# HybridRobotics/ilqr-iterative-tasks

Measured on AMD Instinct MI355X. Metric: batched iLQR iterations/s (n=6,m=2,N=20), higher is better.
Workload: dtype f64

## Files before the change

ilqr_iterative_tasks_amd/csrc/i2lqr_abi.hip:

```cpp
#include <hip/hip_runtime.h>
#include <dlfcn.h>
#include <rccl/rccl.h>

#include <atomic>
#include <cmath>
#include <cstdarg>
#include <cstdio>
#include <cstdlib>
#include <cstring>
#include <mutex>
#include <new>
#include <unordered_set>

#include "../../include/i2lqr.h"
#include "i2lqr_devcfg.hpp"
#include "i2lqr_geometry.hpp"
#include "i2lqr_group.h"
#include "i2lqr_lane.hpp"
#include "i2lqr_select.hpp"
#include "i2lqr_wave.hpp"

#include "i2lqr_lane12.h"

#define I2LQR_DRY_RUN_LANE 1
// ... 354 lines not shown
      return;
    }
  }
  f(std::false_type());
}

template <class T>
IterArgs<T> iter_args(int64_t B, int n_iters, int early_exit, void* X, void* U, const void* x_term,
                      void* lamb, const void* obs, void* cost, void* K, void* k, int32_t* iters,
                      int32_t* status) {
  IterArgs<T> a;
  a.B = B; a.n_iters = n_iters; a.early_exit = early_exit;
  a.X = (T*)X; a.U = (T*)U; a.x_term = (const T*)x_term; a.lamb = (T*)lamb; a.obs = (const T*)obs;
  a.cost = (T*)cost; a.K = (T*)K; a.k = (T*)k; a.iters = iters; a.status = status;
  a.dbg = nullptr;
  a.count = nullptr; a.count_max = 0; a.max_total = 0; a.set_stride = 0;
  return a;
}

template <class T, class Sys> struct Launch {
  static constexpr int n = Sys::n, m = Sys::m, LANES = 64;
  using Cfg = DevCfg<T, n, m>;

  static size_t lds_bytes(int N) { return (size_t)Layout<Sys>(N).total * sizeof(T) * (64 / LANES); }
  static size_t fstep_lds_bytes(int N) {
    return (size_t)Layout<Sys>(N, true).total * sizeof(T) * (64 / LANES);
  }
  static constexpr bool kHasFstep = Sys::n <= 6;
  static unsigned grid(int64_t B) { return (unsigned)((B + (64 / LANES) - 1) / (64 / LANES)); }

  static int prepare(i2lqr_handle* h) {
    h->lanes = LANES;
    h->lds_bytes = lds_bytes(h->cfg.N);
    if (h->lds_bytes > h->geo.max_dyn_lds)
      return fail(I2LQR_ERR_UNSUPPORTED, "horizon %d needs %zu B of LDS per wavefront (> %zu KiB)",
                  h->cfg.N, h->lds_bytes, h->geo.max_dyn_lds / 1024);
    if (h->lds_bytes > h->geo.default_dyn_lds)
      for (const void* kernel :
           {(const void*)k_iterate<T, Sys, LANES, false>, (const void*)k_iterate<T, Sys, LANES, true>,
            (const void*)k_backward<T, Sys, LANES, false>, (const void*)k_backward<T, Sys, LANES, true>,
            (const void*)k_forward<T, Sys, LANES, false>, (const void*)k_forward<T, Sys, LANES, true>,
            (const void*)k_rollout<T, Sys, LANES, false>, (const void*)k_rollout<T, Sys, LANES, true>})
        HIP_TRY(hipFuncSetAttribute(kernel, hipFuncAttributeMaxDynamicSharedMemorySize,
                                    (int)h->lds_bytes));
    return I2LQR_OK;
  }

  static int iterate(i2lqr_handle* h, int64_t B, int n_iters, int early_exit, void* X, void* U,
                     const void* x_term, void* lamb, const void* obs, void* cost, void* K, void* k,
                     int32_t* iters, int32_t* status, hipStream_t s) {
    const Cfg c = make_dev_cfg<T, n, m>(h->cfg);
    IterArgs<T> a = iter_args<T>(B, n_iters, early_exit, X, U, x_term, lamb, obs, cost, K, k, iters,
                                 status);
#ifdef I2LQR_STAMPS
    a.dbg = (unsigned long long*)h->ws;
#endif
    const char* why = "";
    const FusedKernel fk = select_fused(h, B, early_exit != 0, &why);
    if (t_epi && (fk == K_GROUP || fk == K_GROUP16 || fk == K_GROUP_WS)) {
      a.qfun = t_epi->qfun;
      a.outer_iter = t_epi->outer_iter;
      a.max_relax_iter = t_epi->max_relax_iter;
      a.cost_it = (T*)t_epi->cost_it;
      if (t_epi->best_idx) {
        a.pick_part = (MinPair<T>*)t_epi->part;
        a.pick_ticket = h->ticket + h->ticket_next.fetch_add(1, std::memory_order_relaxed) %
                                        i2lqr_handle::kTickets;
        a.best_idx = t_epi->best_idx;
        a.best_cost = (T*)t_epi->best_cost;
      }
      t_epi->fused = true;
    }
    switch (fk) {
      case K_INVALID:
        return fail(I2LQR_ERR_UNSUPPORTED, "%s", why);
      case K_SPEC:
      case K_SPEC16:
        if constexpr (m == 2 && n + m <= 8) {
          HIP_TRY(group_spec_iterate<T>(h->cfg, a, s, fk == K_SPEC16 ? 16 : 8));
          return I2LQR_OK;
        }
        break;
      case K_GROUP:
        if constexpr (m == 2 && n + m <= 8) {
          HIP_TRY(group_iterate<T>(h->cfg, a, s));
          return I2LQR_OK;
        }
        break;
      case K_GROUP16:
        if constexpr (m == 2 && n + m <= 8) {
          HIP_TRY(group16_iterate<T>(h->cfg, a, s, h->opt_group_overlap != 0));
          return I2LQR_OK;
        }
        break;
      case K_GROUP_WS:
        if constexpr (m == 2 && n + m <= 8) {
          HIP_TRY(group_iterate_ws<T>(h->cfg, a, h->ws, s));
          return I2LQR_OK;
        }
        break;
      case K_QUAD:
        if constexpr (n + m == 16) {
          HIP_TRY(quad_iterate<T>(h->cfg, a, h->ws, s));
          return I2LQR_OK;
        }
        break;
      case K_WAVE:
        break;
    }
    const size_t lds_f = fstep_lds_bytes(h->cfg.N);
    const int64_t waves_per_cu = (grid(B) + h->geo.cus - 1) / h->geo.cus;
    const bool fstep = kHasFstep && lds_f <= h->geo.default_dyn_lds &&
                       (h->opt_fstep >= 0 ? h->opt_fstep != 0
                                          : waves_per_cu * lds_f <= h->geo.lds_per_cu - 10 * 1024);
    if constexpr (kHasFstep) {
      if (fstep) {
        with_weights(c.flags, [&](auto W) {
          hipLaunchKernelGGL((k_iterate<T, Sys, LANES, W, true>), dim3(grid(B)), dim3(64), lds_f, s, c, a);
        });
        HIP_TRY(hipGetLastError());
        return I2LQR_OK;
      }
    }
    with_weights(c.flags, [&](auto W) {
      hipLaunchKernelGGL((k_iterate<T, Sys, LANES, W>), dim3(grid(B)), dim3(64), h->lds_bytes, s, c, a);
    });
    HIP_TRY(hipGetLastError());
    return I2LQR_OK;
  }
  static int names_pair(i2lqr_handle*, int64_t, int) { return 0; }
  static int solve_chained(i2lqr_handle* h, int64_t L, int k, void* X, void* U, const void* x_term,
                           void* lamb, const void* obs, void* cost, void* K, void* kk, int32_t* iters,
                           int32_t* status, hipStream_t s) {
    if constexpr (m == 2 && n + m <= 8) {
      if (h->opt_spec == 0 || h->opt_group == 8 || h->opt_group == 64 ||
          !group_spec_chain_supported(h->cfg, L))
        return fail(I2LQR_ERR_UNSUPPORTED, "chains run on the sixteen-lane speculative kernel: a "
                    "bicycle plant with Q = R = 0, at most %lld chains, a horizon whose three-wavefront "
                    "buffers fit a CU's LDS (solve the chain steps one after the other instead)",
                    (long long)h->geo.scaled(512));
      IterArgs<T> a = iter_args<T>(L, h->cfg.max_iter, 1, X, U, x_term, lamb, obs, cost, K, kk, iters,
                                   status);
      a.chain_len = k;
      HIP_TRY(group_spec_chain<T>(h->cfg, a, s));
// ... 949 lines not shown
      if (cfg->Q[i * I2LQR_MAX_N + j] != cfg->Q[j * I2LQR_MAX_N + i] ||
          cfg->Qt[i * I2LQR_MAX_N + j] != cfg->Qt[j * I2LQR_MAX_N + i]) lane_ok = false;
  for (int a = 0; a < cfg->m; a++)
    for (int b = 0; b < cfg->m; b++)
      if (cfg->R[a * I2LQR_MAX_M + b] != cfg->R[b * I2LQR_MAX_M + a]) lane_ok = false;
  int64_t from;
  switch (cfg->system_id) {
    case I2LQR_SYS_BICYCLE4:
    case I2LQR_SYS_BICYCLE6:
      from = weights ? kLaneFromWeights
                     : (early_exit ? lane_from(*cfg).solve : lane_from(*cfg).iterate);
      break;
    case I2LQR_SYS_QUAD12: {
      const LaneFrom q = kLaneFromQuad[cfg->N <= 31 ? 0 : 1][cfg->dtype == I2LQR_F64 ? 0 : 1];
      from = weights ? kLaneFromWeights : (early_exit ? q.solve : q.iterate);
      if (cfg->dtype != I2LQR_F64 && weights) lane_ok = false;
      break;
    }
    default: return fail(I2LQR_ERR_INVALID, "unknown system_id %d", cfg->system_id);
  }
  from = device_geometry().scaled_from(from);
  if (!lane_ok || B < from) return I2LQR_LAYOUT_PROBLEM_MAJOR;
  return B % 64 == 0 ? I2LQR_LAYOUT_BATCH_TILED : I2LQR_LAYOUT_BATCH_MINOR;
}

int i2lqr_set_compaction(i2lqr_handle* h, int64_t min_batch) {
  if (!h) return fail(I2LQR_ERR_INVALID, "null handle");
  if (h->cfg.layout == I2LQR_LAYOUT_PROBLEM_MAJOR && min_batch > 0)
    return fail(I2LQR_ERR_UNSUPPORTED, "compaction applies to the batch-minor / batch-tiled layouts");
  h->compact_min_batch = min_batch < 0 ? -1 : min_batch;
  return I2LQR_OK;
}

int i2lqr_set_option(i2lqr_handle* h, const char* name, int64_t value) {
  if (!h || !name) return fail(I2LQR_ERR_INVALID, "null handle or option name");
  if (value < -1 || value > 0x7fffffff) return fail(I2LQR_ERR_INVALID, "option value out of range");
  const int v = (int)value;
  if (!strcmp(name, "defer_states")) h->opt_defer = v < 0 ? -1 : (v != 0);
  else if (!strcmp(name, "reroll_nominal")) h->opt_reroll = v < 0 ? -1 : (v != 0);
  else if (!strcmp(name, "lds_gain_steps")) h->opt_lds_steps = v;
  else if (!strcmp(name, "merge_inputs")) h->opt_merge = v < 0 ? -1 : (v != 0);
  else if (!strcmp(name, "checkpoint_states")) h->opt_ckpt = v < 0 ? -1 : (v != 0);
  else if (!strcmp(name, "stagger")) h->opt_stagger = v;
  else if (!strcmp(name, "per_step_jacobians")) h->opt_fstep = v < 0 ? -1 : (v != 0);
  else if (!strcmp(name, "wave_tail")) h->wave_tail = v < 0 ? -1 : (v > 65536 ? 65536 : v);
  else if (!strcmp(name, "first_chunk")) h->opt_first_chunk = v < 1 ? -1 : (v > 1024 ? 1024 : v);
  else if (!strcmp(name, "helper_wavefront")) h->opt_pair = v < 0 ? -1 : (v != 0);
  else if (!strcmp(name, "state_buffers")) h->opt_two_x = v < 0 ? -1 : (v != 0);
  else if (!strcmp(name, "chunk_step")) h->opt_chunk_step = v < 1 ? -1 : (v > 1024 ? 1024 : v);
  else if (!strcmp(name, "fused_compaction")) h->opt_fuse = v < 0 ? -1 : (v != 0);
  else if (!strcmp(name, "final_round")) h->opt_final_round = v < 0 ? -1 : (v > 20 ? 20 : v);
  else if (!strcmp(name, "speculate")) h->opt_spec = v < 0 ? -1 : (v != 0);
  else if (!strcmp(name, "group_workspace")) h->opt_group_ws = v < 0 ? -1 : (v != 0);
  else if (!strcmp(name, "group_overlap")) h->opt_group_overlap = v < 0 ? -1 : (v != 0);
  else if (!strcmp(name, "debug_self_test")) {
#ifdef I2LQR_DEBUG
    unsigned long long* w = i2lqr::debug_trap_word();
    double* buf = nullptr;
    HIP_TRY(hipMalloc((void**)&buf, 8 * sizeof(double)));
    hipLaunchKernelGGL(k_debug_self_test, dim3(1), dim3(64), 0, (hipStream_t)0, buf, w);
    const int rc = debug_check(I2LQR_OK, nullptr);
    (void)hipFree(buf);
    return rc;
#else
    return fail(I2LQR_ERR_UNSUPPORTED, "\"debug_self_test\" exists in the index-checked debug build "
                "only (make -C ilqr_iterative_tasks_amd/csrc debug)");
#endif
  }
  else if (!strcmp(name, "group_lanes")) {
    if (v != -1 && v != 8 && v != 16 && v != 64)
      return fail(I2LQR_ERR_INVALID, "\"group_lanes\" is 8, 16, 64 or -1");
    h->opt_group = v;
  }
  else return fail(I2LQR_ERR_INVALID, "unknown option '%s'", name);
  return I2LQR_OK;
}

static const char* kernel_name(const i2lqr_handle* h, int64_t B, bool early_exit) {
  if (!h) return "";
  if (h->cfg.layout != I2LQR_LAYOUT_PROBLEM_MAJOR) {
    if (h->cfg.system_id == I2LQR_SYS_QUAD12) return "k_lane_iterate_rows";
    const auto pair = [&](auto L) {
      return L.names_pair(const_cast<i2lqr_handle*>(h), B, early_exit ? 1 : 0);
    };
    return dispatch(h, pair) == 1 ? "k_lane_iterate_pair" : "k_lane_iterate";
  }
  switch (select_fused(h, B, early_exit, nullptr)) {
    case K_SPEC: return "k_group_spec";
    case K_SPEC16: return "k_group_spec (sixteen lanes)";
    case K_GROUP: return "k_group_iterate";
    case K_GROUP16: return "k_group_iterate (sixteen lanes)";
    case K_GROUP_WS: return "k_group_iterate (workspace form)";
    case K_QUAD: return "k_quad_iterate";
    case K_WAVE: return "k_iterate";
    default: return "unsupported";
  }
}

const char* i2lqr_iterate_kernel(const i2lqr_handle* h, int64_t B) { return kernel_name(h, B, false); }
const char* i2lqr_solve_kernel(const i2lqr_handle* h, int64_t B) { return kernel_name(h, B, true); }

int i2lqr_set_workspace(i2lqr_handle* h, void* workspace, int64_t bytes) {
  if (!h) return fail(I2LQR_ERR_INVALID, "null handle");
  if (bytes < 0 || (bytes > 0 && !workspace) || ((uintptr_t)workspace & 15))
    return fail(I2LQR_ERR_INVALID, "workspace must be a 16-byte aligned device pointer");
  h->ws = workspace;
  h->ws_bytes = bytes;
// ... 558 lines not shown
```

ilqr_iterative_tasks_amd/csrc/i2lqr_group.h:

```cpp
#pragma once
#include <hip/hip_runtime.h>

#include "../../include/i2lqr.h"
#include "i2lqr_wave.hpp"

namespace i2lqr {

bool group_supported(const i2lqr_config& cfg);
template <class T> hipError_t group_iterate(const i2lqr_config& cfg, const IterArgs<T>& a,
                                            hipStream_t stream);

constexpr int64_t kGroup16Batch = 4096;
bool group16_supported(const i2lqr_config& cfg);
template <class T> hipError_t group16_iterate(const i2lqr_config& cfg, const IterArgs<T>& a,
                                              hipStream_t stream, bool overlap = true);

constexpr int64_t kGroupWsBatch = 4096;
constexpr int64_t kGroupWsTop = 8192;
constexpr int64_t kGroupWsTopF32 = 7168;
inline int64_t group_ws_top(const i2lqr_config& cfg) {
  return cfg.dtype == I2LQR_F64 ? kGroupWsTop : kGroupWsTopF32;
}
int64_t group_workspace_bytes(const i2lqr_config& cfg, int64_t B);
template <class T> hipError_t group_iterate_ws(const i2lqr_config& cfg, const IterArgs<T>& a,
                                               void* ws, hipStream_t stream);

bool group_spec_supported(const i2lqr_config& cfg, int lanes);
template <class T> hipError_t group_spec_iterate(const i2lqr_config& cfg, const IterArgs<T>& a,
                                                 hipStream_t stream, int lanes);
bool group_spec_chain_supported(const i2lqr_config& cfg, int64_t chains);
template <class T> hipError_t group_spec_chain(const i2lqr_config& cfg, const IterArgs<T>& a,
                                               hipStream_t stream);
bool group_spec_tail_supported(const i2lqr_config& cfg);
template <class T> hipError_t group_spec_tail(const i2lqr_config& cfg, const IterArgs<T>& a,
                                              hipStream_t stream);

bool quad_supported(const i2lqr_config& cfg);
int64_t quad_workspace_bytes(const i2lqr_config& cfg, int64_t B);
template <class T> hipError_t quad_iterate(const i2lqr_config& cfg, const IterArgs<T>& a, void* ws,
                                           hipStream_t stream);

}
```

ilqr_iterative_tasks_amd/csrc/i2lqr_group.hip:

```cpp
#include "i2lqr_group.h"

#include "i2lqr_devcfg.hpp"
#include "i2lqr_geometry.hpp"
#include "i2lqr_group.hpp"
#include "i2lqr_dryrun.hpp"

namespace i2lqr {

namespace {

template <class T, class Sys, int G = kGroup> size_t group_lds_bytes(int N) {
  return (size_t)GLayout<Sys, G>(N).wave_words() * sizeof(T);
}

template <auto Kernel> hipError_t raise_lds_limit(size_t lds) {
  if (lds <= device_geometry().default_dyn_lds) return hipSuccess;
  constexpr int kMaxDev = 64;
  static thread_local int raised_for[kMaxDev] = {};
  int dev = 0;
  hipError_t e = hipGetDevice(&dev);
  if (e != hipSuccess) return e;
  if (dev < 0 || dev >= kMaxDev || raised_for[dev] < (int)lds) {
    e = hipFuncSetAttribute((const void*)Kernel, hipFuncAttributeMaxDynamicSharedMemorySize,
                            (int)lds);
    if (e != hipSuccess) return e;
    if (dev >= 0 && dev < kMaxDev) raised_for[dev] = (int)lds;
  }
  return hipSuccess;
}

template <class T, class Sys, int H, int G = kGroup>
hipError_t launch_h(const i2lqr_config& cfg, const IterArgs<T>& a, hipStream_t s) {
  const auto c = make_dev_cfg<T, Sys::n, Sys::m>(cfg);
  const size_t lds = group_lds_bytes<T, Sys, G>(cfg.N);
  if (hipError_t e = raise_lds_limit<k_group_iterate<T, Sys, H, false, G>>(lds); e != hipSuccess)
    return e;
  constexpr int PW = 64 / G;
  const unsigned grid = (unsigned)((a.B + PW - 1) / PW);
  hipLaunchKernelGGL((k_group_iterate<T, Sys, H, false, G>), dim3(grid), dim3(64 * H), lds, s, c, a,
                     (T*)nullptr);
  return hipGetLastError();
}
template <class T, class Sys>
hipError_t launch16(const i2lqr_config& cfg, const IterArgs<T>& a, hipStream_t s, bool overlap) {
  const int64_t cus = device_geometry().cus;
#ifndef I2LQR_STAMPS
  if (overlap && (a.B + 3) / 4 <= cus) return launch_h<T, Sys, 3, 16>(cfg, a, s);
  if ((a.B + 3) / 4 <= 2 * cus) return launch_h<T, Sys, 2, 16>(cfg, a, s);
#endif
  return launch_h<T, Sys, 1, 16>(cfg, a, s);
}
template <class T, class Sys>
hipError_t launch_ws(const i2lqr_config& cfg, const IterArgs<T>& a, void* ws, hipStream_t s) {
  const auto c = make_dev_cfg<T, Sys::n, Sys::m>(cfg);
  const size_t lds = (size_t)GLayout<Sys>(cfg.N, true).wave_words() * sizeof(T);
  if (hipError_t e = raise_lds_limit<k_group_iterate<T, Sys, 1, true>>(lds); e != hipSuccess) return e;
  const unsigned grid = (unsigned)((a.B + kGroupsPerWave - 1) / kGroupsPerWave);
  hipLaunchKernelGGL((k_group_iterate<T, Sys, 1, true>), dim3(grid), dim3(64), lds, s, c, a, (T*)ws);
  return hipGetLastError();
}

template <class T, class Sys>
hipError_t launch(const i2lqr_config& cfg, const IterArgs<T>& a, hipStream_t s) {
  const int64_t cus = device_geometry().cus;
#ifndef I2LQR_STAMPS
  if ((a.B + kGroupsPerWave - 1) / kGroupsPerWave <= cus) return launch_h<T, Sys, 3>(cfg, a, s);
#endif
  return launch_h<T, Sys, 1>(cfg, a, s);
}

constexpr int kSpecWideBatch = 512;

template <class T, class Sys, int V, int G = kGroup> size_t spec_lds_bytes(int N) {
  return (size_t)GSpecLayout<Sys, V, G>(N).group_words() * sizeof(T);
}

template <class T, class Sys, int V, bool SETIO, int G>
hipError_t launch_spec_v(const i2lqr_config& cfg, const IterArgs<T>& a, hipStream_t s) {
  const auto c = make_dev_cfg<T, Sys::n, Sys::m>(cfg);
  const size_t lds = spec_lds_bytes<T, Sys, V, G>(cfg.N);
  if (hipError_t e = raise_lds_limit<k_group_spec<T, Sys, V, SETIO, G>>(lds); e != hipSuccess)
    return e;
  constexpr int PW = 64 / G;
  const int64_t problems = SETIO ? (int64_t)a.count_max : a.B;
  const unsigned grid = (unsigned)((problems + PW - 1) / PW);
  hipLaunchKernelGGL((k_group_spec<T, Sys, V, SETIO, G>), dim3(grid), dim3(64 * V), lds, s, c, a);
  return hipGetLastError();
}
template <class T, class Sys, bool SETIO, int G>
hipError_t launch_spec(const i2lqr_config& cfg, const IterArgs<T>& a, hipStream_t s) {
  const DeviceGeometry& geo = device_geometry();
  const bool wide = !SETIO && a.B <= geo.scaled(kSpecWideBatch) &&
                    spec_lds_bytes<T, Sys, 3, G>(cfg.N) <= geo.max_dyn_lds;
  if (wide) return launch_spec_v<T, Sys, 3, SETIO, G>(cfg, a, s);
  return launch_spec_v<T, Sys, 2, SETIO, G>(cfg, a, s);
}
template <class T, bool SETIO>
hipError_t launch_spec_any(const i2lqr_config& cfg, const IterArgs<T>& a, hipStream_t s, int lanes) {
  return visit_bicycle<T>(cfg, [&](auto, auto sys) {
    using Sys = decltype(sys);
// ... 18 lines not shown
    return group_lds_bytes<decltype(t), decltype(sys), G>(cfg.N);
  });
  return lds <= device_geometry().max_dyn_lds;
}

}

bool group_spec_supported(const i2lqr_config& cfg, int lanes) {
  if (!spec_plant_ok(cfg) || cfg.layout != I2LQR_LAYOUT_PROBLEM_MAJOR) return false;
  return lanes == 16 ? spec_lds_fits<16>(cfg) : (group_supported(cfg) && spec_lds_fits<kGroup>(cfg));
}
int group_spec_tail_lanes(const i2lqr_config& cfg) {
  if (!spec_plant_ok(cfg)) return 0;
  return spec_lds_fits<16>(cfg) ? 16 : (spec_lds_fits<kGroup>(cfg) ? kGroup : 0);
}
bool group_spec_tail_supported(const i2lqr_config& cfg) { return group_spec_tail_lanes(cfg) != 0; }

template <class T, class Sys>
hipError_t launch_spec_chain(const i2lqr_config& cfg, const IterArgs<T>& a, hipStream_t s) {
  const auto c = make_dev_cfg<T, Sys::n, Sys::m>(cfg);
  const size_t lds = spec_lds_bytes<T, Sys, 3, 16>(cfg.N);
  if (hipError_t e = raise_lds_limit<k_group_spec<T, Sys, 3, false, 16, true>>(lds); e != hipSuccess)
    return e;
  const unsigned grid = (unsigned)((a.B + 3) / 4);
  hipLaunchKernelGGL((k_group_spec<T, Sys, 3, false, 16, true>), dim3(grid), dim3(64 * 3), lds, s, c, a);
  return hipGetLastError();
}
bool group_spec_chain_supported(const i2lqr_config& cfg, int64_t chains) {
  if (!spec_plant_ok(cfg) || cfg.layout != I2LQR_LAYOUT_PROBLEM_MAJOR) return false;
  const DeviceGeometry& geo = device_geometry();
  if (chains > geo.scaled(kSpecWideBatch)) return false;
  const size_t lds = visit_bicycle(cfg, [&](auto t, auto sys) {
    return spec_lds_bytes<decltype(t), decltype(sys), 3, 16>(cfg.N);
  });
  return lds <= geo.max_dyn_lds;
}
template <class T>
hipError_t group_spec_chain(const i2lqr_config& cfg, const IterArgs<T>& a, hipStream_t s) {
  return visit_bicycle<T>(cfg, [&](auto, auto sys) {
    return launch_spec_chain<T, decltype(sys)>(cfg, a, s);
  });
}
template <class T>
hipError_t group_spec_iterate(const i2lqr_config& cfg, const IterArgs<T>& a, hipStream_t s, int lanes) {
  return launch_spec_any<T, false>(cfg, a, s, lanes);
}
template <class T>
hipError_t group_spec_tail(const i2lqr_config& cfg, const IterArgs<T>& a, hipStream_t s) {
  return launch_spec_any<T, true>(cfg, a, s, group_spec_tail_lanes(cfg));
}

bool group16_supported(const i2lqr_config& cfg) { return group_lds_fits<16>(cfg); }
template <class T>
hipError_t group16_iterate(const i2lqr_config& cfg, const IterArgs<T>& a, hipStream_t s, bool overlap) {
  return visit_bicycle<T>(cfg, [&](auto, auto sys) {
    return launch16<T, decltype(sys)>(cfg, a, s, overlap);
  });
}

bool group_supported(const i2lqr_config& cfg) { return group_lds_fits<kGroup>(cfg); }

int64_t group_workspace_bytes(const i2lqr_config& cfg, int64_t B) {
  if (!group_supported(cfg) || B <= 0) return 0;
  const int64_t probs = (B + kGroupsPerWave - 1) / kGroupsPerWave * kGroupsPerWave;
  const int64_t words = visit_bicycle<double>(cfg, [&](auto, auto sys) {
    return GLayout<decltype(sys)>(cfg.N, true).ws_words();
  });
  const size_t lds = visit_bicycle(cfg, [&](auto t, auto sys) {
    return (size_t)GLayout<decltype(sys)>(cfg.N, true).wave_words() * sizeof(t);
  });
  if (lds > device_geometry().max_dyn_lds) return 0;
  return probs * words * (cfg.dtype == I2LQR_F64 ? 8 : 4);
}
template <class T>
hipError_t group_iterate_ws(const i2lqr_config& cfg, const IterArgs<T>& a, void* ws, hipStream_t s) {
  return visit_bicycle<T>(cfg, [&](auto, auto sys) {
    return launch_ws<T, decltype(sys)>(cfg, a, ws, s);
  });
}

template <class T>
hipError_t group_iterate(const i2lqr_config& cfg, const IterArgs<T>& a, hipStream_t s) {
  return visit_bicycle<T>(cfg, [&](auto, auto sys) { return launch<T, decltype(sys)>(cfg, a, s); });
}

#define I2LQR_GROUP_LAUNCHERS(T)                                                                    \
  template hipError_t group_iterate<T>(const i2lqr_config&, const IterArgs<T>&, hipStream_t);       \
  template hipError_t group16_iterate<T>(const i2lqr_config&, const IterArgs<T>&, hipStream_t, bool); \
  template hipError_t group_iterate_ws<T>(const i2lqr_config&, const IterArgs<T>&, void*,           \
                                          hipStream_t);                                             \
  template hipError_t group_spec_iterate<T>(const i2lqr_config&, const IterArgs<T>&, hipStream_t,   \
                                            int);                                                   \
  template hipError_t group_spec_chain<T>(const i2lqr_config&, const IterArgs<T>&, hipStream_t);    \
  template hipError_t group_spec_tail<T>(const i2lqr_config&, const IterArgs<T>&, hipStream_t);
I2LQR_GROUP_LAUNCHERS(double)
I2LQR_GROUP_LAUNCHERS(float)

}
```

ilqr_iterative_tasks_amd/csrc/i2lqr_group.hpp:

```cpp
#pragma once
#include <hip/hip_runtime.h>
#include <stdint.h>

#include "i2lqr_systems.hpp"
#include "i2lqr_wave.hpp"

namespace i2lqr {

constexpr int kGroup = 8;
constexpr int kGroupsPerWave = 64 / kGroup;

template <class Sys> struct GroupPattern {
  static constexpr int n = Sys::n, m = Sys::m, W = n + m, NV = Sys::NVAR;
  static constexpr int dt_row(int b) {
    for (int i = 2; i < n; i++)
      if (i != b && Sys::pat(i, b) == 2) return i;
    return -1;
  }
  static constexpr bool column_ok(int b) {
    int extra = 0;
    for (int i = 0; i < n; i++) {
      const int code = Sys::pat(i, b);
      if (i < 2) {
        if (code == 2) return false;
// ... 245 lines not shown
    const T spd_y = opt == 1 ? ob[4] : T(0), spd_x = opt == 2 ? ob[4] : T(0);
    const int rounds = (N + stride) / stride;
    for (int r = 0; r < rounds; r++) {
      const int t0 = first + r * stride;
      const int t = t0 < N ? t0 : N;
      const int ts = t0 < N ? t0 : N - 1;
      T* Rs = rec(ts);
      {
        T xe[n], tr[NT], u[m], jv[NV];
#pragma unroll
        for (int i = 0; i < n; i++) xe[i] = S[XUo + (ts + 1) * W + i];
#pragma unroll
        for (int a = 0; a < m; a++) u[a] = S[XUo + ts * W + n + a];
#pragma unroll
        for (int q = 0; q < NT; q++) tr[q] = S[TRo + (ts + 1) * NT + q];
        Sys::jac_var(c, xe, u, tr, jv);
#pragma unroll
        for (int q = 0; q < NV; q++) Rs[GL::R_JV + q] = jv[q];
#pragma unroll
        for (int a = 0; a < m; a++) {
          T e_hi, e_lo;
          if (sizeof(T) == 8 && c.fast_barrier) {
            e_hi = t_exp_bounded(c.ctrl_q2 * (u[a] - c.u_max[a]));
            e_lo = c.ctrl_c[a] * t_rcp(e_hi);
          } else {
            e_hi = t_exp(c.ctrl_q2 * (u[a] - c.u_max[a]));
            e_lo = t_exp(c.ctrl_q2 * (-c.u_max[a] - u[a]));
          }
          Rs[GL::R_LU + a] = c.ctrl_q12 * e_hi - c.ctrl_q12 * e_lo;
          Rs[GL::R_LUU + a] = c.ctrl_q122 * e_hi +
                              c.ctrl_q122 * e_lo;
        }
      }
      T* R = rec(t);
      R[GL::R_ZERO] = T(0);
      R[GL::R_ONE] = T(1);
      const T px = S[XUo + t * W + 0], py = S[XUo + t * W + 1];
      const T dz = opt == 2 ? px - (ob[0] - T(t) * spd_x) : px - ob[0];
      const T dy = opt == 1 ? py - (ob[1] + T(t) * spd_y) : py - ob[1];
      const T h = T(1) + c.safety_margin - (dz * pa * dz + dy * pb * dy);
      const T hd0 = T(-2) * pa * dz, hd1 = T(-2) * pb * dy;
      const T e = t_exp(c.obs_q2 * h);
      const T c1 = c.obs_q12 * e, c2 = c.obs_q122 * e;
      R[GL::R_OB + 0] = has_ob ? c1 * hd0 : T(0);
      R[GL::R_OB + 1] = has_ob ? c1 * hd1 : T(0);
      R[GL::R_OB + 2] = has_ob ? c2 * (hd0 * hd0) : T(0);
      R[GL::R_OB + 3] = has_ob ? c2 * (hd0 * hd1) : T(0);
      R[GL::R_OB + 4] = has_ob ? c2 * (hd1 * hd1) : T(0);
    }
    wave_sync();
    ws_publish();
  }

  __device__ __forceinline__ void quu_inverse(const T (&Quu)[m * m], T lamb, T (&inv)[m * m]) const {
    static_assert(m == 2, "the eight-lane kernel is written for m == 2 plants");
    t_quu_inverse2(Quu, lamb, inv);
  }

  template <bool GENERAL>
  __device__ __forceinline__ bool backward(int XUo, const T (&xT)[n], T lamb, bool commit) const {
    if constexpr (G == 16) return backward_row<GENERAL>(XUo, xT, lamb, commit);
    bool bad = false;
    T va[n];
    {
      const T* Rn = rec(N);
      T dx[n];
#pragma unroll
      for (int i = 0; i < n; i++) dx[i] = S[XUo + N * W + i] - xT[i];
#pragma unroll
      for (int i = 0; i < n; i++) {
        T vxx = T(0), vx = T(0);
#pragma unroll
        for (int r = 0; r < n; r++) {
          const T q = T(2) * Qt[i * n + r];
          vxx = (g == r) ? q : vxx;
          vx += q * dx[r];
        }
        va[i] = (g == n) ? vx : vxx;
      }
      va[0] += Rn[off_l0];
      va[1] += Rn[off_l1];
    }
    const int gcol = g < GL::KW ? g : GL::KW - 1;
    struct Rec { T jv[NV], luu[m], c0, c1, l0, l1, lrow[m]; };
    Rec ra, rb;
    auto load_record = [&](int t, Rec& r) __attribute__((always_inline)) {
      const T* R = rec(t);
#pragma unroll
      for (int q = 0; q < NV; q++) r.jv[q] = R[GL::R_JV + q];
#pragma unroll
      for (int a = 0; a < m; a++) r.luu[a] = R[GL::R_LUU + a];
      r.c0 = R[off_c0];
      r.c1 = R[off_c1];
      r.l0 = R[off_l0];
      r.l1 = R[off_l1];
#pragma unroll
      for (int a = 0; a < m; a++) r.lrow[a] = R[off_lu[a]];
    };
    load_record(N - 1, ra);
    auto step = [&](const int t, Rec& rc, Rec& rn) __attribute__((always_inline)) {
      if constexpr (WS) load_record(t > 0 ? t - 1 : 0, rn);
      const T (&jv)[NV] = rc.jv;
      const T (&luu)[m] = rc.luu;
      const T (&lrow)[m] = rc.lrow;
      const T c0 = rc.c0, c1 = rc.c1, l0 = rc.l0, l1 = rc.l1;
      STAMP_BEGIN();
// ... 86 lines not shown
      for (int a = 0; a < m; a++) {
        T acc = T(0);
#pragma unroll
        for (int b = 0; b < m; b++) acc = t_fma(Quu[a * m + b], kc[b], acc);
        qk[a] = acc;
      }
#pragma unroll
      for (int i = 0; i < n; i++) {
        T acc = T(0);
#pragma unroll
        for (int a = 0; a < m; a++) acc = t_fma(kr[a][i], qk[a], acc);
        va[i] = h[i] - acc;
      }
      STAMP_END(5);
    };
    int t = N - 1;
    if constexpr (I2LQR_GROUP_UNROLL >= 4) {
      for (; t >= 3; t -= 4) {
        step(t, ra, rb);
        step(t - 1, rb, ra);
        step(t - 2, ra, rb);
        step(t - 3, rb, ra);
      }
    }
    for (; t >= 1; t -= 2) {
      step(t, ra, rb);
      step(t - 1, rb, ra);
    }
    if (t == 0) step(0, ra, rb);
    ws_publish();
    return bad;
  }

  template <bool GENERAL>
  __device__ __forceinline__ bool backward_row(int XUo, const T (&xT)[n], T lamb, bool commit) const {
    T vb[n];
    terminal_base(XUo, xT, vb);
    return backward_row_from<GENERAL>(vb, lamb, commit);
  }
  __device__ __forceinline__ void terminal_base(int XUo, const T (&xT)[n], T (&vb)[n]) const {
    T dx[n];
#pragma unroll
    for (int i = 0; i < n; i++) dx[i] = S[XUo + N * W + i] - xT[i];
    const int gq = g < n ? g : 0;
#pragma unroll
    for (int i = 0; i < n; i++) {
      T vx = T(0);
#pragma unroll
      for (int r = 0; r < n; r++) vx += (T(2) * Qt[i * n + r]) * dx[r];
      const T vxx = T(2) * Qt[i * n + gq];
      vb[i] = (g == n) ? vx : (g < n ? vxx : T(0));
    }
  }
  template <bool GENERAL>
  __device__ __forceinline__ bool backward_row_from(const T (&vb)[n], T lamb, bool commit) const {
    static_assert(GL::KW > n + 1, "the padding word of a gain row takes the stores of idle lanes");
    bool bad = false;
    T va[n];
    {
      const T* Rn = rec(N);
#pragma unroll
      for (int i = 0; i < n; i++) va[i] = vb[i];
      va[0] += Rn[off_l0];
      va[1] += Rn[off_l1];
    }
    const int gcol = (commit && g <= n) ? g : GL::KW - 1;
    T cdr[n];
#pragma unroll
    for (int r = 0; r < n; r++) cdr[r] = (rsrc == r) ? cdt : T(0);
    struct Rec { T jv[NV], luu[m], c0, c1, l0, l1, lrow[m]; };
    Rec ra, rb;
    auto load_record = [&](int t, Rec& r) __attribute__((always_inline)) {
      const T* R = rec(t);
#pragma unroll
      for (int q = 0; q < NV; q++) r.jv[q] = R[GL::R_JV + q];
#pragma unroll
      for (int a = 0; a < m; a++) r.luu[a] = R[GL::R_LUU + a];
      r.c0 = R[off_c0];
      r.c1 = R[off_c1];
      r.l0 = R[off_l0];
      r.l1 = R[off_l1];
#pragma unroll
      for (int a = 0; a < m; a++) r.lrow[a] = R[off_lu[a]];
    };
    auto f_entry = [&](auto k_, auto b_, const T (&jv)[NV]) __attribute__((always_inline)) {
      constexpr int code = Sys::pat(decltype(k_)::value, n + decltype(b_)::value);
      if constexpr (code == 1) return T(1);
      else if constexpr (code == 2) return c.dt;
      else return jv[code >= 3 ? code - 3 : 0];
    };
    load_record(N - 1, ra);
    auto step = [&](const int t, Rec& rc, Rec& rn) __attribute__((always_inline)) {
      const T (&jv)[NV] = rc.jv;
      T t1[W];
      static_for_i<0, W>([&](auto a_) {
        constexpr int a = decltype(a_)::value;
        T acc = T(0);
        bool first = true;
        static_for_i<0, n>([&](auto i_) {
          constexpr int i = decltype(i_)::value;
          f_acc<i, a>(acc, first, va[i], jv);
        });
        t1[a] = acc;
      });
      dpp_ready(t1);
      load_record(t > 0 ? t - 1 : 0, rn);
      T Quu[m * m], Qinv[m * m];
      {
// ... 25 lines not shown
          constexpr int r = decltype(r_)::value;
          constexpr bool used = [] {
            for (int b = 0; b < n; b++)
              if (GP::dt_row(b) == r) return true;
            return false;
          }();
          if constexpr (used) bcast_fmac<r>(hr, src, cdr[r]);
        });
      };
      T hu[m], hx[n];
      h_rows(std::integral_constant<int, n>{}, hu);
#pragma unroll
      for (int a = 0; a < m; a++) hu[a] += rc.lrow[a];
      if constexpr (GENERAL) quu_inverse(Quu, lamb, Qinv);
      else t_quu_inverse2_pd(Quu, lamb, Qinv, &bad);
      h_rows(std::integral_constant<int, 0>{}, hx);
      hx[0] += rc.l0;
      hx[1] += rc.l1;
      T pk[m], kc[m];
#pragma unroll
      for (int a = 0; a < m; a++) {
        T acc = T(0);
#pragma unroll
        for (int b = 0; b < m; b++) acc = t_fma(Qinv[a * m + b], hu[b], acc);
        pk[a] = acc;
        kc[a] = -acc;
      }
      T* Kt = gain_x(t);
#pragma unroll
      for (int a = 0; a < m; a++) Kt[a * GL::KW + gcol] = kc[a];
      T qk[m];
#pragma unroll
      for (int a = 0; a < m; a++) {
        T acc = T(0);
#pragma unroll
        for (int b = 0; b < m; b++) acc = t_fma(Quu[a * m + b], kc[b], acc);
        qk[a] = acc;
      }
      T vn[n];
#pragma unroll
      for (int i = 0; i < n; i++) vn[i] = hx[i];
      static_for_i<0, n>([&](auto i_) {
        constexpr int i = decltype(i_)::value;
#pragma unroll
        for (int a = 0; a < m; a++) bcast_fmac1<i>(vn[i], pk[a], qk[a]);
      });
#pragma unroll
      for (int i = 0; i < n; i++) va[i] = vn[i];
    };
    STAMP_BEGIN();
    int t = N - 1;
    if constexpr (I2LQR_GROUP_UNROLL >= 4) {
      for (; t >= 3; t -= 4) {
        step(t, ra, rb);
        step(t - 1, rb, ra);
        step(t - 2, ra, rb);
        step(t - 3, rb, ra);
      }
    }
    for (; t >= 1; t -= 2) {
      step(t, ra, rb);
      step(t - 1, rb, ra);
    }
    if (t == 0) step(0, ra, rb);
    STAMP_END(1);
    wave_sync();
    return bad;
  }

  __device__ __forceinline__ T forward_row(int XUo, int XUn, int TRn, const T (&xT)[n],
                                           bool* bad) const {
    static_assert(G == 16 && m == 2, "two inputs on the two halves of a 16-lane row");
    const int half = g >> 3;
    const T umax = half ? c.u_max[1] : c.u_max[0];
    T x[n], u[m], xn[n], tr[NT];
#pragma unroll
    for (int i = 0; i < n; i++) x[i] = S[XUo + i];
#pragma unroll
    for (int i = 0; i < n; i++) S[XUn + i] = x[i];
    Sys::template trig_g<false>(x, tr, bad);
#pragma unroll
    for (int q = 0; q < NT; q++) S[TRn + q] = tr[q];
    static_assert(!WS, "gain rows and records are neighbours in the LDS slice");
    auto pXo = S + XUo;
    auto pXn = S + XUn;
    auto pG = S + (oKk + half * GL::KW);
    auto pTR = S + (TRn + half * NT);
    T xo[n], uo, kk[NA];
    auto load_step = [&](auto k_) __attribute__((always_inline)) {
      constexpr int k = decltype(k_)::value;
#pragma unroll
      for (int j = 0; j < n; j++) xo[j] = pXo[k * W + j];
      uo = pXo[k * W + n + half];
#pragma unroll
      for (int j = 0; j < NA; j++) kk[j] = pG[k * (m * GL::KW) + j];
    };
    load_step(std::integral_constant<int, 0>{});
    auto step = [&](auto k_, const T (&trc)[NT]) __attribute__((always_inline)) {
      constexpr int k = decltype(k_)::value;
      T acc = T(0);
#pragma unroll
      for (int j = 0; j < n; j++) acc = t_fma(kk[j], x[j] - xo[j], acc);
      const T ua = clip(uo + kk[n] + acc, -umax, umax);
      load_step(std::integral_constant<int, k + 1>{});
      pXn[k * W + n + half] = ua;
      u[0] = bcast_mov<0>(ua);
// ... 78 lines not shown
        load_step(t + 1 < N ? t + 1 : t, qn);
      } else {
        load_step(t + 1 < N ? t + 1 : t, q);
      }
#pragma unroll
      for (int a = 0; a < m; a++) S[XUn + t * W + n + a] = u[a];
      Sys::template trig_g<GENERAL>(x, tr, bad);
#pragma unroll
      for (int q = 0; q < NT; q++) S[TRn + t * NT + q] = tr[q];
      Sys::step_tr(c, x, u, tr, xn);
#pragma unroll
      for (int i = 0; i < n; i++) S[XUn + (t + 1) * W + i] = xn[i];
#pragma unroll
      for (int i = 0; i < n; i++) x[i] = xn[i];
    };
    int t = 0;
    if constexpr (WS) {
      for (; t + 1 < N; t += 2) {
        step(t, ga, gb);
        step(t + 1, gb, ga);
      }
      if (t < N) step(t, ga, gb);
    } else {
      if constexpr (I2LQR_GROUP_UNROLL >= 4) {
        for (; t + 3 < N; t += 4) {
          step(t, ga, ga);
          step(t + 1, ga, ga);
          step(t + 2, ga, ga);
          step(t + 3, ga, ga);
        }
      }
      for (; t + 1 < N; t += 2) {
        step(t, ga, ga);
        step(t + 1, ga, ga);
      }
      if (t < N) step(t, ga, ga);
    }
    Sys::template trig_g<GENERAL>(x, tr, bad);
#pragma unroll
    for (int q = 0; q < NT; q++) S[TRn + N * NT + q] = tr[q];
    const T cost = terminal_cost(x, xT);
    wave_sync();
    return cost;
  }
};

__device__ __forceinline__ int idx_div(int e, int d, float rcp_d) {
  int q = (int)((float)e * rcp_d);
  const int r = e - q * d;
  q += (r >= d) ? 1 : 0;
  q -= (r < 0) ? 1 : 0;
  return q;
}

template <class T, class Sys, int H = 1, bool WS = false, int G = kGroup>
__global__ __launch_bounds__(64 * H) void k_group_iterate(const DevCfg<T, Sys::n, Sys::m> c,
                                                          const IterArgs<T> a, T* ws = nullptr) {
  static_assert(!(WS && H > 1), "the workspace form runs without helper wavefronts");
  constexpr int n = Sys::n, m = Sys::m, W = n + m;
#ifdef I2LQR_STAMPS
  constexpr bool OVL = false;
#else
  constexpr bool OVL = G == 16 && H >= 3;
#endif
  using GL = GLayout<Sys, G>;
  extern __shared__ __align__(16) unsigned char gsmem_raw[];
  T* smem = reinterpret_cast<T*>(gsmem_raw);
  const int lane = threadIdx.x & 63, hv = threadIdx.x >> 6;
#ifdef I2LQR_STAMPS
  unsigned long long st_k0, st_k1, st_k2, st_k3;
  asm volatile("s_memtime %0\n\ts_waitcnt lgkmcnt(0)" : "=s"(st_k0)::"memory");
#endif
  const int64_t prob0 = (int64_t)blockIdx.x * GL::PW + lane / G;
  const bool real = prob0 < a.B;
  const int64_t prob = real ? prob0 : a.B - 1;
  GroupWorker<T, Sys, WS, G> w(c, smem, lane);
  const int N = c.N, g = w.g;
  const float rN = 1.0f / (float)N, rN1 = 1.0f / (float)(N + 1), rnN = 1.0f / (float)(n * N);
  const GL& L = w.L;
  const auto S = w.S;
  if constexpr (WS) w.Wp = ws + prob0 * (int64_t)L.ws_words();

  if (H == 1 || hv == 0) {
    const T* gX = a.X + prob * (int64_t)(n * (N + 1));
    if (g < n) S[L.XU0 + g] = gX[g * (N + 1)];
    const T* gU = a.U + prob * (int64_t)(m * N);
    for (int e = g; e < m * N; e += G) {
      const int aa = idx_div(e, N, rN), t = e - aa * N;
      S[L.XU0 + t * W + n + aa] = gU[e];
    }
    for (int e = lane; e < n * n; e += 64) smem[L.qt_base() + e] = c.Qt[e];
  }
  T xT[n], ob[6];
#pragma unroll
  for (int i = 0; i < n; i++) xT[i] = a.x_term[prob * n + i];
#pragma unroll
  for (int q = 0; q < 6; q++) ob[q] = a.obs ? a.obs[prob * 6 + q] : T(q == 5 ? -1 : 1);
  T lamb = a.lamb[prob];
  wave_sync();

  int cur = 0;
  const T ob_pa = T(1) / (ob[2] * ob[2]), ob_pb = T(1) / (ob[3] * ob[3]);
  int* const ctl = reinterpret_cast<int*>(smem + L.ctl_base());
  if constexpr (H > 1) {
    if (hv > 0) {
      const int h0 = OVL ? hv - 1 : hv, hs = OVL ? H - 1 : H;
      for (;;) {
        __syncthreads();
        const int flags = ctl[8];
        if (!(flags & 1)) break;
        if (flags & 2) {
          const int pc = ctl[lane / G];
          w.prep(pc ? L.XU1 : L.XU0, pc ? L.TR1 : L.TR0, ob, ob_pa, ob_pb, h0 * G + g, hs * G);
        }
        __syncthreads();
      }
      if constexpr (OVL) {
        if (real && a.K) {
          T* const gK = a.K + prob * (int64_t)(m * n * N);
          T* const gk = a.k + prob * (int64_t)(m * N);
          for (int t = h0 * G + g; t < N; t += hs * G) {
            const T* Kt = w.gain(t);
            T kv[m][n + 1];
#pragma unroll
            for (int aa = 0; aa < m; aa++)
#pragma unroll
              for (int j = 0; j <= n; j++) kv[aa][j] = Kt[aa * GL::KW + j];
#pragma unroll
            for (int aa = 0; aa < m; aa++) {
#pragma unroll
              for (int j = 0; j < n; j++) gK[(aa * n + j) * N + t] = kv[aa][j];
              gk[aa * N + t] = kv[aa][n];
            }
          }
        }
      }
      return;
    }
  }
  T vb[n];
#pragma unroll
  for (int i = 0; i < n; i++) vb[i] = T(0);
  T cost = w.rollout(L.XU0, L.TR0, xT);
  int it = 0, status = a.early_exit ? 2  : 0 ;
  T cost_ret = cost;
  bool fresh = true, active = a.n_iters > 0;
#ifdef I2LQR_STAMPS
  asm volatile("s_memtime %0\n\ts_waitcnt lgkmcnt(0)" : "=s"(st_k1)::"memory");
#endif
  while (__any(active)) {
    const int XUo = cur ? L.XU1 : L.XU0, XUn = cur ? L.XU0 : L.XU1;
    const int TRo = cur ? L.TR1 : L.TR0, TRn = cur ? L.TR0 : L.TR1;
#ifdef I2LQR_STAMPS
    {
      auto& st_t0 = w.st_t0; auto& st_t1 = w.st_t1; auto& st_acc = w.st_acc;
      STAMP_BEGIN();
      if (__any(fresh)) w.prep(XUo, TRo, ob, ob_pa, ob_pb, g, G);
      STAMP_END(0);
    }
#else
    if constexpr (H > 1) {
      const bool do_prep = __any(fresh);
      if (g == 0) ctl[lane / G] = cur;
      if (lane == 0) ctl[8] = 1 | (do_prep ? 2 : 0);
      __syncthreads();
      if constexpr (OVL) {
        if (do_prep) w.terminal_base(XUo, xT, vb);
      } else {
        if (do_prep) w.prep(XUo, TRo, ob, ob_pa, ob_pb, g, H * G);
      }
      __syncthreads();
    } else {
      if (__any(fresh)) w.prep(XUo, TRo, ob, ob_pa, ob_pb, g, G);
    }
#endif
    if constexpr (OVL) {
      if (__builtin_expect(__any(w.template backward_row_from<false>(vb, lamb, active)), 0))
        w.template backward_row_from<true>(vb, lamb, active);
    } else {
      if (__builtin_expect(__any(w.template backward<false>(XUo, xT, lamb, active)), 0))
        w.template backward<true>(XUo, xT, lamb, active);
    }
    T cost_new;
    {
#ifdef I2LQR_STAMPS
      auto& st_t0 = w.st_t0; auto& st_t1 = w.st_t1; auto& st_acc = w.st_acc;
      STAMP_BEGIN();
#endif
      bool big = false;
      cost_new = w.template forward<false>(XUo, XUn, TRn, xT, &big);
      if (__builtin_expect(__any(big), 0)) cost_new = w.template forward<true>(XUo, XUn, TRn, xT, &big);
#ifdef I2LQR_STAMPS
      STAMP_END(6);
#endif
    }
    {
      const bool acc = active && cost_new < cost, rej = active && !(cost_new < cost);
      const T lamb_dn = lamb / c.lamb_factor, lamb_up = lamb * c.lamb_factor;
      const bool conv = t_abs((cost_new - cost) / cost) < c.eps;
      it += active ? 1 : 0;
      fresh = acc;
      cur ^= acc ? 1 : 0;
      lamb = acc ? lamb_dn : (rej ? lamb_up : lamb);
      cost_ret = acc ? cost_new : (rej ? cost : cost_ret);
      cost = acc ? cost_new : cost;
      const bool stop_conv = acc && conv, stop_lamb = rej && lamb > c.max_lamb;
      const int ended = stop_conv ? 1 : 3;
      if (a.early_exit) {
        status = (stop_conv || stop_lamb) ? ended : status;
        active = active && !(stop_conv || stop_lamb);
      } else {
        status = (status == 0 && (stop_conv || stop_lamb)) ? ended : status;
      }
      active = active && it < a.n_iters;
    }
  }
#ifdef I2LQR_STAMPS
  asm volatile("s_memtime %0\n\ts_waitcnt lgkmcnt(0)" : "=s"(st_k2)::"memory");
#endif
  if constexpr (H > 1) {
    if (lane == 0) ctl[8] = 0;
    __syncthreads();
  }
  if (!t_isfinite(cost_ret)) status = 4;

  if (OVL && real) {
    const int XUo = cur ? L.XU1 : L.XU0;
    T* const gX = a.X + prob * (int64_t)(n * (N + 1));
    T* const gU = a.U + prob * (int64_t)(m * N);
    for (int t = g; t <= N; t += G) {
      T xu[W];
#pragma unroll
      for (int i = 0; i < W; i++) xu[i] = S[XUo + t * W + i];
#pragma unroll
      for (int i = 0; i < n; i++) gX[i * (N + 1) + t] = xu[i];
      if (t < N) {
#pragma unroll
        for (int aa = 0; aa < m; aa++) gU[aa * N + t] = xu[n + aa];
      }
    }
    if (g == 0) {
      a.lamb[prob] = lamb;
      a.cost[prob] = cost_ret;
      if (a.iters) a.iters[prob] = it;
      if (a.status) a.status[prob] = status;
    }
  }
  if (!OVL && real) {
    const int XUo = cur ? L.XU1 : L.XU0;
    T* gX = a.X + prob * (int64_t)(n * (N + 1));
    for (int e = g; e < n * (N + 1); e += G) {
      const int i = idx_div(e, N + 1, rN1), t = e - i * (N + 1);
      gX[e] = S[XUo + t * W + i];
    }
    T* gU = a.U + prob * (int64_t)(m * N);
    for (int e = g; e < m * N; e += G) {
      const int aa = idx_div(e, N, rN), t = e - aa * N;
      gU[e] = S[XUo + t * W + n + aa];
    }
    if (a.K) {
      T* gK = a.K + prob * (int64_t)(m * n * N);
      for (int e = g; e < m * n * N; e += G) {
        const int aa = idx_div(e, n * N, rnN), r = e - aa * (n * N);
        const int j = idx_div(r, N, rN), t = r - j * N;
        gK[e] = w.gain(t)[aa * GL::KW + j];
      }
      T* gk = a.k + prob * (int64_t)(m * N);
      for (int e = g; e < m * N; e += G) {
        const int aa = idx_div(e, N, rN), t = e - aa * N;
        gk[e] = w.gain(t)[aa * GL::KW + n];
      }
// ... 271 lines not shown
```

Measured before the change: 75.21 million.

## Add four-wavefront group16 overlap that splits prep across helper wavefronts

Adds an H=4 variant of the group16 overlapped kernel. Three helper wavefronts split the per-iteration prep work: one computes control-barrier terms for input 0, one for input 1, and one computes state Jacobians and obstacle terms. Prep runs in two chunks, and the main wavefront joins the second chunk through a barrier placed mid-way through the backward pass, so it only waits for the first chunk before starting. This mode becomes the default when the batch fits within the CU count. It also adds optional per-round timestamp instrumentation, at the cost of a larger workgroup, an extra barrier per round and a remapped lane layout for the helpers.

```diff
diff --git a/ilqr_iterative_tasks_amd/csrc/i2lqr_abi.hip b/ilqr_iterative_tasks_amd/csrc/i2lqr_abi.hip
--- a/ilqr_iterative_tasks_amd/csrc/i2lqr_abi.hip
+++ b/ilqr_iterative_tasks_amd/csrc/i2lqr_abi.hip
@@ -430,7 +430,7 @@
     const Cfg c = make_dev_cfg<T, n, m>(h->cfg);
     IterArgs<T> a = iter_args<T>(B, n_iters, early_exit, X, U, x_term, lamb, obs, cost, K, k, iters,
                                  status);
-#ifdef I2LQR_STAMPS
+#if defined(I2LQR_STAMPS) || defined(I2LQR_ROUND_STAMPS)
     a.dbg = (unsigned long long*)h->ws;
 #endif
     const char* why = "";
@@ -467,7 +467,7 @@
         break;
       case K_GROUP16:
         if constexpr (m == 2 && n + m <= 8) {
-          HIP_TRY(group16_iterate<T>(h->cfg, a, s, h->opt_group_overlap != 0));
+          HIP_TRY(group16_iterate<T>(h->cfg, a, s, h->opt_group_overlap < 0 ? 2 : h->opt_group_overlap));
           return I2LQR_OK;
         }
         break;
@@ -1523,7 +1523,7 @@
   else if (!strcmp(name, "final_round")) h->opt_final_round = v < 0 ? -1 : (v > 20 ? 20 : v);
   else if (!strcmp(name, "speculate")) h->opt_spec = v < 0 ? -1 : (v != 0);
   else if (!strcmp(name, "group_workspace")) h->opt_group_ws = v < 0 ? -1 : (v != 0);
-  else if (!strcmp(name, "group_overlap")) h->opt_group_overlap = v < 0 ? -1 : (v != 0);
+  else if (!strcmp(name, "group_overlap")) h->opt_group_overlap = v < 0 ? -1 : (v > 2 ? 2 : v);
   else if (!strcmp(name, "debug_self_test")) {
 #ifdef I2LQR_DEBUG
     unsigned long long* w = i2lqr::debug_trap_word();
diff --git a/ilqr_iterative_tasks_amd/csrc/i2lqr_group.h b/ilqr_iterative_tasks_amd/csrc/i2lqr_group.h
--- a/ilqr_iterative_tasks_amd/csrc/i2lqr_group.h
+++ b/ilqr_iterative_tasks_amd/csrc/i2lqr_group.h
@@ -13,7 +13,7 @@
 constexpr int64_t kGroup16Batch = 4096;
 bool group16_supported(const i2lqr_config& cfg);
 template <class T> hipError_t group16_iterate(const i2lqr_config& cfg, const IterArgs<T>& a,
-                                              hipStream_t stream, bool overlap = true);
+                                              hipStream_t stream, int overlap = 2);
 
 constexpr int64_t kGroupWsBatch = 4096;
 constexpr int64_t kGroupWsTop = 8192;
diff --git a/ilqr_iterative_tasks_amd/csrc/i2lqr_group.hip b/ilqr_iterative_tasks_amd/csrc/i2lqr_group.hip
--- a/ilqr_iterative_tasks_amd/csrc/i2lqr_group.hip
+++ b/ilqr_iterative_tasks_amd/csrc/i2lqr_group.hip
@@ -42,10 +42,11 @@
   return hipGetLastError();
 }
 template <class T, class Sys>
-hipError_t launch16(const i2lqr_config& cfg, const IterArgs<T>& a, hipStream_t s, bool overlap) {
+hipError_t launch16(const i2lqr_config& cfg, const IterArgs<T>& a, hipStream_t s, int overlap) {
   const int64_t cus = device_geometry().cus;
 #ifndef I2LQR_STAMPS
-  if (overlap && (a.B + 3) / 4 <= cus) return launch_h<T, Sys, 3, 16>(cfg, a, s);
+  if (overlap >= 2 && (a.B + 3) / 4 <= cus) return launch_h<T, Sys, 4, 16>(cfg, a, s);
+  if (overlap == 1 && (a.B + 3) / 4 <= cus) return launch_h<T, Sys, 3, 16>(cfg, a, s);
   if ((a.B + 3) / 4 <= 2 * cus) return launch_h<T, Sys, 2, 16>(cfg, a, s);
 #endif
   return launch_h<T, Sys, 1, 16>(cfg, a, s);
@@ -170,7 +171,7 @@
 
 bool group16_supported(const i2lqr_config& cfg) { return group_lds_fits<16>(cfg); }
 template <class T>
-hipError_t group16_iterate(const i2lqr_config& cfg, const IterArgs<T>& a, hipStream_t s, bool overlap) {
+hipError_t group16_iterate(const i2lqr_config& cfg, const IterArgs<T>& a, hipStream_t s, int overlap) {
   return visit_bicycle<T>(cfg, [&](auto, auto sys) {
     return launch16<T, decltype(sys)>(cfg, a, s, overlap);
   });
@@ -204,7 +205,7 @@
 
 #define I2LQR_GROUP_LAUNCHERS(T)                                                                    \
   template hipError_t group_iterate<T>(const i2lqr_config&, const IterArgs<T>&, hipStream_t);       \
-  template hipError_t group16_iterate<T>(const i2lqr_config&, const IterArgs<T>&, hipStream_t, bool); \
+  template hipError_t group16_iterate<T>(const i2lqr_config&, const IterArgs<T>&, hipStream_t, int);  \
   template hipError_t group_iterate_ws<T>(const i2lqr_config&, const IterArgs<T>&, void*,           \
                                           hipStream_t);                                             \
   template hipError_t group_spec_iterate<T>(const i2lqr_config&, const IterArgs<T>&, hipStream_t,   \
diff --git a/ilqr_iterative_tasks_amd/csrc/i2lqr_group.hpp b/ilqr_iterative_tasks_amd/csrc/i2lqr_group.hpp
--- a/ilqr_iterative_tasks_amd/csrc/i2lqr_group.hpp
+++ b/ilqr_iterative_tasks_amd/csrc/i2lqr_group.hpp
@@ -321,6 +321,63 @@
     ws_publish();
   }
 
+  template <int a> __device__ __forceinline__ void prep_input(int XUo, int k0, int k1) const {
+    for (int k = k0; k < k1; k += G) {
+      const int ts = k < N ? N - 1 - k : 0;
+      T* Rs = rec(ts);
+      const T u = S[XUo + ts * W + n + a];
+      T e_hi, e_lo;
+      if (sizeof(T) == 8 && c.fast_barrier) {
+        e_hi = t_exp_bounded(c.ctrl_q2 * (u - c.u_max[a]));
+        e_lo = c.ctrl_c[a] * t_rcp(e_hi);
+      } else {
+        e_hi = t_exp(c.ctrl_q2 * (u - c.u_max[a]));
+        e_lo = t_exp(c.ctrl_q2 * (-c.u_max[a] - u));
+      }
+      Rs[GL::R_LU + a] = c.ctrl_q12 * e_hi - c.ctrl_q12 * e_lo;
+      Rs[GL::R_LUU + a] = c.ctrl_q122 * e_hi +
+                          c.ctrl_q122 * e_lo;
+    }
+  }
+  __device__ __forceinline__ void prep_state(int XUo, int TRo, const T (&ob)[6], T pa, T pb, int k0,
+                                             int k1) const {
+    const bool has_ob = ob[5] >= T(0);
+    const int opt = has_ob ? (int)ob[5] : 0;
+    const T spd_y = opt == 1 ? ob[4] : T(0), spd_x = opt == 2 ? ob[4] : T(0);
+    for (int k = k0; k < k1; k += G) {
+      const int t = k <= N ? N - k : 0;
+      const int ts = t < N ? t : N - 1;
+      T* Rs = rec(ts);
+      {
+        T xe[n], tr[NT], u[m], jv[NV];
+#pragma unroll
+        for (int i = 0; i < n; i++) xe[i] = S[XUo + (ts + 1) * W + i];
+#pragma unroll
+        for (int a = 0; a < m; a++) u[a] = S[XUo + ts * W + n + a];
+#pragma unroll
+        for (int q = 0; q < NT; q++) tr[q] = S[TRo + (ts + 1) * NT + q];
+        Sys::jac_var(c, xe, u, tr, jv);
+#pragma unroll
+        for (int q = 0; q < NV; q++) Rs[GL::R_JV + q] = jv[q];
+      }
+      T* R = rec(t);
+      R[GL::R_ZERO] = T(0);
+      R[GL::R_ONE] = T(1);
+      const T px = S[XUo + t * W + 0], py = S[XUo + t * W + 1];
+      const T dz = opt == 2 ? px - (ob[0] - T(t) * spd_x) : px - ob[0];
+      const T dy = opt == 1 ? py - (ob[1] + T(t) * spd_y) : py - ob[1];
+      const T h = T(1) + c.safety_margin - (dz * pa * dz + dy * pb * dy);
+      const T hd0 = T(-2) * pa * dz, hd1 = T(-2) * pb * dy;
+      const T e = t_exp(c.obs_q2 * h);
+      const T c1 = c.obs_q12 * e, c2 = c.obs_q122 * e;
+      R[GL::R_OB + 0] = has_ob ? c1 * hd0 : T(0);
+      R[GL::R_OB + 1] = has_ob ? c1 * hd1 : T(0);
+      R[GL::R_OB + 2] = has_ob ? c2 * (hd0 * hd0) : T(0);
+      R[GL::R_OB + 3] = has_ob ? c2 * (hd0 * hd1) : T(0);
+      R[GL::R_OB + 4] = has_ob ? c2 * (hd1 * hd1) : T(0);
+    }
+  }
+
   __device__ __forceinline__ void quu_inverse(const T (&Quu)[m * m], T lamb, T (&inv)[m * m]) const {
     static_assert(m == 2, "the eight-lane kernel is written for m == 2 plants");
     t_quu_inverse2(Quu, lamb, inv);
@@ -513,8 +570,12 @@
       vb[i] = (g == n) ? vx : (g < n ? vxx : T(0));
     }
   }
-  template <bool GENERAL>
-  __device__ __forceinline__ bool backward_row_from(const T (&vb)[n], T lamb, bool commit) const {
+  struct NoMid { __device__ __forceinline__ void operator()() const {} };
+  template <bool GENERAL, class Mid = NoMid>
+  __device__ __forceinline__ bool backward_row_from(const T (&vb)[n], T lamb, bool commit,
+                                                    Mid mid = Mid()) const {
+    static_assert(std::is_same_v<Mid, NoMid> || I2LQR_GROUP_UNROLL >= 4,
+                  "mid() sits between the first two groups of four steps");
     static_assert(GL::KW > n + 1, "the padding word of a gain row takes the stores of idle lanes");
     bool bad = false;
     T va[n];
@@ -646,6 +707,9 @@
     int t = N - 1;
     if constexpr (I2LQR_GROUP_UNROLL >= 4) {
       for (; t >= 3; t -= 4) {
+        if constexpr (!std::is_same_v<Mid, NoMid>) {
+          if (t == N - 5) mid();
+        }
         step(t, ra, rb);
         step(t - 1, rb, ra);
         step(t - 2, ra, rb);
@@ -830,6 +894,19 @@
   q -= (r < 0) ? 1 : 0;
   return q;
 }
+
+#ifdef I2LQR_ROUND_STAMPS
+#define ROUND_STAMP(v)                                                          \
+  do {                                                                          \
+    __builtin_amdgcn_sched_barrier(0);                                          \
+    asm volatile("s_memtime %0\n\ts_waitcnt lgkmcnt(0)" : "=s"(v)::"memory"); \
+    __builtin_amdgcn_sched_barrier(0);                                          \
+  } while (0)
+#define ROUND_SUM(slot, d) (rs_acc[slot] += (d))
+#else
+#define ROUND_STAMP(v)
+#define ROUND_SUM(slot, d)
+#endif
 
 template <class T, class Sys, int H = 1, bool WS = false, int G = kGroup>
 __global__ __launch_bounds__(64 * H) void k_group_iterate(const DevCfg<T, Sys::n, Sys::m> c,
@@ -841,10 +918,13 @@
 #else
   constexpr bool OVL = G == 16 && H >= 3;
 #endif
+  constexpr bool PART = OVL && H == 4;
   using GL = GLayout<Sys, G>;
   extern __shared__ __align__(16) unsigned char gsmem_raw[];
   T* smem = reinterpret_cast<T*>(gsmem_raw);
-  const int lane = threadIdx.x & 63, hv = threadIdx.x >> 6;
+  const int hv = threadIdx.x >> 6;
+  const int lane = (PART && hv > 0) ? (threadIdx.x & 3) * G + ((threadIdx.x & 63) >> 2)
+                                    : (threadIdx.x & 63);
 #ifdef I2LQR_STAMPS
   unsigned long long st_k0, st_k1, st_k2, st_k3;
   asm volatile("s_memtime %0\n\ts_waitcnt lgkmcnt(0)" : "=s"(st_k0)::"memory");
@@ -883,10 +963,27 @@
   if constexpr (H > 1) {
     if (hv > 0) {
       const int h0 = OVL ? hv - 1 : hv, hs = OVL ? H - 1 : H;
+      const int k_end = (N + G) / G * G;
       for (;;) {
         __syncthreads();
         const int flags = ctl[8];
         if (!(flags & 1)) break;
+        if constexpr (PART) {
+          const int pc = ctl[lane / G];
+          const int XUo = pc ? L.XU1 : L.XU0, TRo = pc ? L.TR1 : L.TR0;
+          auto part = [&](int k0, int k1) __attribute__((always_inline)) {
+            if (hv == 1) w.template prep_input<0>(XUo, k0, k1);
+            else if (hv == 2) w.template prep_input<1>(XUo, k0, k1);
+            else w.prep_state(XUo, TRo, ob, ob_pa, ob_pb, k0, k1);
+          };
+          if (flags & 2) part(g, G);
+          __syncthreads();
+          if ((flags & 2) && k_end > G) {
+            part(G + g, k_end);
+            __syncthreads();
+          }
+          continue;
+        }
         if (flags & 2) {
           const int pc = ctl[lane / G];
           w.prep(pc ? L.XU1 : L.XU0, pc ? L.TR1 : L.TR0, ob, ob_pa, ob_pb, h0 * G + g, hs * G);
@@ -923,12 +1020,17 @@
   int it = 0, status = a.early_exit ? 2  : 0 ;
   T cost_ret = cost;
   bool fresh = true, active = a.n_iters > 0;
+#ifdef I2LQR_ROUND_STAMPS
+  unsigned long long rs_acc[8] = {0, 0, 0, 0, 0, 0, 0, 0}, rs_t0 = 0, rs_t1 = 0, rs_t2 = 0, rs_l0 = 0;
+  ROUND_STAMP(rs_l0);
+#endif
 #ifdef I2LQR_STAMPS
   asm volatile("s_memtime %0\n\ts_waitcnt lgkmcnt(0)" : "=s"(st_k1)::"memory");
 #endif
   while (__any(active)) {
     const int XUo = cur ? L.XU1 : L.XU0, XUn = cur ? L.XU0 : L.XU1;
     const int TRo = cur ? L.TR1 : L.TR0, TRn = cur ? L.TR0 : L.TR1;
+    [[maybe_unused]] bool join_b3 = false;
 #ifdef I2LQR_STAMPS
     {
       auto& st_t0 = w.st_t0; auto& st_t1 = w.st_t1; auto& st_acc = w.st_acc;
@@ -941,18 +1043,36 @@
       const bool do_prep = __any(fresh);
       if (g == 0) ctl[lane / G] = cur;
       if (lane == 0) ctl[8] = 1 | (do_prep ? 2 : 0);
+      ROUND_STAMP(rs_t0);
       __syncthreads();
       if constexpr (OVL) {
         if (do_prep) w.terminal_base(XUo, xT, vb);
       } else {
         if (do_prep) w.prep(XUo, TRo, ob, ob_pa, ob_pb, g, H * G);
       }
+      ROUND_STAMP(rs_t1);
       __syncthreads();
+      ROUND_STAMP(rs_t2);
+      ROUND_SUM(0, do_prep ? rs_t2 - rs_t0 : 0);
+      ROUND_SUM(1, do_prep ? rs_t2 - rs_t1 : 0);
+      ROUND_SUM(3, do_prep ? 1 : 0);
+      join_b3 = PART && do_prep && N >= G;
     } else {
       if (__any(fresh)) w.prep(XUo, TRo, ob, ob_pa, ob_pb, g, G);
     }
 #endif
-    if constexpr (OVL) {
+    if constexpr (PART) {
+      auto b3 = [&]() __attribute__((always_inline)) {
+        if (join_b3) {
+          ROUND_STAMP(rs_t1);
+          __syncthreads();
+          ROUND_STAMP(rs_t2);
+          ROUND_SUM(2, rs_t2 - rs_t1);
+        }
+      };
+      if (__builtin_expect(__any(w.template backward_row_from<false>(vb, lamb, active, b3)), 0))
+        w.template backward_row_from<true>(vb, lamb, active);
+    } else if constexpr (OVL) {
       if (__builtin_expect(__any(w.template backward_row_from<false>(vb, lamb, active)), 0))
         w.template backward_row_from<true>(vb, lamb, active);
     } else {
@@ -995,6 +1115,13 @@
   }
 #ifdef I2LQR_STAMPS
   asm volatile("s_memtime %0\n\ts_waitcnt lgkmcnt(0)" : "=s"(st_k2)::"memory");
+#endif
+#ifdef I2LQR_ROUND_STAMPS
+  ROUND_STAMP(rs_t0);
+  rs_acc[4] = rs_t0 - rs_l0;
+  rs_acc[5] = (unsigned long long)it;
+  if (H > 1 && real && a.dbg && g == 0)
+    for (int q = 0; q < 8; q++) a.dbg[prob * 8 + q] = rs_acc[q];
 #endif
   if constexpr (H > 1) {
     if (lane == 0) ctl[8] = 0;
```

Result: slower. 73.06 million (-2.9%).
